# pelinski/TransformerGrooveInfilling

Hardware: AMD Instinct MI355X
Metric: HVO sequences/sec (32-step, d_model=128) per train step (higher is better)
Workload: dtype f32; 1 GPU; BASELINE configs[1]: InfillingClosedHH_training.yaml + overrides d_model=128/4 heads/3 layers, dim_feedforward=512, bs=64 per GPU, dropout=0.24, SGD lr=0.07, hit_loss_penalty=0.38, S=16, encoder-only; global_batch=64, parallelism=dp1, hipgraph=False

## Files before the change

### transformergrooveinfilling_amd/csrc/gt_seq.h

```cpp
#pragma once
#include "gt_seq_api.h"
#include <type_traits>

#ifdef GT_SEQ_STAMPS
#define GT_STAMP(i) do { if (blockIdx.x == 0 && threadIdx.x == 0) reinterpret_cast<long long*>(a.ws + a.stamps)[(i)] = (long long)__builtin_amdgcn_s_memtime(); } while (0)
__shared__ long long* gt_sub_ptr;
#define GT_SUBSTAMP(i) do { if (threadIdx.x == 0 && gt_sub_ptr) gt_sub_ptr[(i)] = (long long)__builtin_amdgcn_s_memtime(); } while (0)
#define GT_SUBWAIT() asm volatile("s_waitcnt vmcnt(0) lgkmcnt(0)" ::: "memory")
#define GT_SUBSET(on) do { if (threadIdx.x == 0) gt_sub_ptr = ((on) && blockIdx.x == 0) ? reinterpret_cast<long long*>(a.ws + a.stamps) + 200 : nullptr; } while (0)
#define GT_WGSTAMP(k) do { if (threadIdx.x == 0 && a.phase == 1 && blockIdx.x < 512) { long long* q_ = reinterpret_cast<long long*>(a.ws + a.stamps) + 1024 + 4 * blockIdx.x + 2 * (k); \
    q_[0] = (long long)__builtin_amdgcn_s_memtime(); q_[1] = (long long)__builtin_amdgcn_s_memrealtime(); } } while (0)
#else
#define GT_WGSTAMP(k) do { } while (0)
#define GT_STAMP(i) do { } while (0)
#define GT_SUBSTAMP(i) do { } while (0)
#define GT_SUBWAIT() do { } while (0)
#define GT_SUBSET(on) do { } while (0)
#endif

#define GT_SEQ_WAVES 8
#define GT_SEQ_NT (GT_SEQ_WAVES * 64)
#define GT_SEQ_NT_WG GT_SEQ_NT
#include "gt_seq_wg.h"

// ... 478 lines not shown
  const int q4 = ncol >> 2;
  for (int e = tid; e < nrows * q4; e += GT_SEQ_NT) {
    const int r = rb + e / q4, c = (e % q4) * 4;
    *reinterpret_cast<float4*>(dst + (unsigned)(r * ncol + c)) = *reinterpret_cast<const float4*>(sT + r * str + c);
  }
}

__device__ __forceinline__ void seq_tile_out_cols(float* __restrict__ dst, const int ldd, const float* sT, const int str, const int c0, const int ncol,
                                                  const int tid, const int rb, const int nrows) {
  const int q4 = ncol >> 2;
  for (int e = tid; e < nrows * q4; e += GT_SEQ_NT) {
    const int r = rb + e / q4, c = c0 + (e % q4) * 4;
    *reinterpret_cast<float4*>(dst + (unsigned)(r * ldd + c)) = *reinterpret_cast<const float4*>(sT + r * str + c);
  }
}

template <int CW> struct SeqLnPre { float ga[CW], be[CW], bi[CW]; };
template <int CW>
__device__ __forceinline__ void seq_ln_pre(SeqLnPre<CW>& p, const float* __restrict__ bias, const float* __restrict__ gamma, const float* __restrict__ beta,
                                           const int tid) {
  const int c0 = (tid & 15) * CW;
  SeqVec<CW>::ld(p.ga, gamma + c0); SeqVec<CW>::ld(p.be, beta + c0); SeqVec<CW>::ld(p.bi, bias + c0);
}
template <int DP, bool HALF, typename ZFun>
__device__ __forceinline__ void seq_ln_fwd(ZFun zfun, float* sY, const int str, const int d, const float* __restrict__ gamma,
                                           const float* __restrict__ beta, float* gy, float* gxhat, float* grstd, const int tid, const int rb,
                                           const SeqLnPre<DP / 16>* pre = nullptr) {
  constexpr int CW = DP / 16;
  if (HALF && tid >= 256) return;
  const int row = rb + (tid >> 4), seg = tid & 15, c0 = seg * CW;
  const bool ok = c0 < d;
  float z[CW], ga[CW], be[CW];
#pragma unroll
  for (int e = 0; e < CW; ++e) { z[e] = 0.f; ga[e] = 0.f; be[e] = 0.f; }
  if (ok) {
    if (pre != nullptr) {
#pragma unroll
      for (int e = 0; e < CW; ++e) { ga[e] = pre->ga[e]; be[e] = pre->be[e]; }
    } else { SeqVec<CW>::ld(ga, gamma + c0); SeqVec<CW>::ld(be, beta + c0); }
    zfun(row, c0, z);
  }
  float s = 0.f;
#pragma unroll
  for (int e = 0; e < CW; ++e) s += z[e];
  const float invd = 1.0f / (float)d, mean = seq_row16_sum(s) * invd;
  float q = 0.f;
  if (ok) {
#pragma unroll
    for (int e = 0; e < CW; ++e) { const float t = z[e] - mean; q += t * t; }
  }
  const float rs = 1.0f / sqrtf(seq_row16_sum(q) * invd + GT_LN_EPS);
  if (ok) {
    float xh[CW], y[CW];
#pragma unroll
    for (int e = 0; e < CW; ++e) { xh[e] = (z[e] - mean) * rs; y[e] = xh[e] * ga[e] + be[e]; }
    const unsigned o = (unsigned)(row * d + c0);
    SeqVec<CW>::st(sY + row * str + c0, y);
    if (gy != nullptr) {
      SeqVec<CW>::st(gy + o, y);
      SeqVec<CW>::st(gxhat + o, xh);
    }
  }
  if (seg == 0 && gy != nullptr) grstd[row] = rs;
}

template <int CW> struct SeqLnBwdPre { float xh[CW], ga[CW], rs; };
template <int CW>
__device__ __forceinline__ void seq_ln_bwd_pre(SeqLnBwdPre<CW>& p, const int d, const float* __restrict__ gxhat, const float* __restrict__ grstd,
                                               const float* __restrict__ gamma, const int tid, const int rb) {
  const int row = rb + ((tid >> 4) & 15), c0 = (tid & 15) * CW;
  SeqVec<CW>::ld(p.xh, gxhat + (unsigned)(row * d + c0)); SeqVec<CW>::ld(p.ga, gamma + c0);
  p.rs = grstd[row];
}
template <int DP, bool HALF, typename GFun>
__device__ __forceinline__ void seq_ln_bwd(GFun gfun, float* sDz, float* sDzm, const int str, const int d, const float* __restrict__ gxhat,
                                           const float* __restrict__ grstd, const float* __restrict__ gamma, const SeqDropK& dk, const uint32_t key,
                                           const uint32_t idx0, float* gdz, float* gdzm, float* sP, const int tid, const int rb,
                                           const SeqLnBwdPre<DP / 16>* pre = nullptr) {
  constexpr int CW = DP / 16;
  if (HALF && tid >= 256) return;
  const int row = rb + (tid >> 4), seg = tid & 15, c0 = seg * CW, lane = tid & 63, wave = tid >> 6;
  const bool ok = c0 < d;
  const unsigned o = (unsigned)(row * d + c0);
  float g[CW], xh[CW], ga[CW];
#pragma unroll
  for (int e = 0; e < CW; ++e) { g[e] = 0.f; xh[e] = 0.f; ga[e] = 0.f; }
  float rs;
  if (pre != nullptr) {
    rs = pre->rs;
#pragma unroll
    for (int e = 0; e < CW; ++e) { xh[e] = pre->xh[e]; ga[e] = pre->ga[e]; }
    if (ok) gfun(row, c0, g);
  } else {
    rs = grstd[row];
    if (ok) { SeqVec<CW>::ld(xh, gxhat + o); SeqVec<CW>::ld(ga, gamma + c0); gfun(row, c0, g); }
  }
  float s1 = 0.f, s2 = 0.f;
#pragma unroll
  for (int e = 0; e < CW; ++e) { const float gd = g[e] * ga[e]; s1 += gd; s2 += gd * xh[e]; }
  const float invd = 1.0f / (float)d, m1 = seq_row16_sum(s1) * invd, m2 = seq_row16_sum(s2) * invd;
  float cg[CW], cb[CW];
#pragma unroll
  for (int e = 0; e < CW; ++e) { cg[e] = g[e] * xh[e]; cb[e] = g[e]; }
#pragma unroll
  for (int e = 0; e < CW; ++e) { cg[e] += __shfl_xor(cg[e], 16); cb[e] += __shfl_xor(cb[e], 16); }
#pragma unroll
  for (int e = 0; e < CW; ++e) { cg[e] += __shfl_xor(cg[e], 32); cb[e] += __shfl_xor(cb[e], 32); }
  if (lane < 16 && ok) { SeqVec<CW>::st(sP + (wave * 2) * DP + c0, cg); SeqVec<CW>::st(sP + (wave * 2 + 1) * DP + c0, cb); }
  if (ok) {
    float v[CW], vm[CW];
// ... 461 lines not shown
#pragma unroll
    for (int c = 0; c < HD; ++c) sQ[ia * ldq + ha * HD + c] = G.dq.v[c];
  }
  if (tid < 2 * nkrow * H) {
    const int pb = tid & 1, jb = krow0 + (tid >> 1) % nkrow, hb = (tid >> 1) / nkrow;
    float* dst = sQ + jb * ldq + (pb ? 2 * d : d) + hb * HD;
#pragma unroll
    for (int c = 0; c < HD; ++c) dst[c] = pb ? G.dvv.v[c] : G.dkk.v[c];
  }
}

__device__ __forceinline__ int seq_vblock(const int bid, const int nper, const int B) {
  if ((B & 7) != 0 || bid >= nper * B) return bid;
  const int xcd = bid & 7, slot = bid >> 3;
  return ((slot / nper) * 8 + xcd) * nper + slot % nper;
}

template <int DP> struct SeqGeo {
  static constexpr int SX = DP + 8, SH = GT_SEQ_FMAX + 8, SQ = 3 * DP + 8, SRS = DP + 8, RP = DP == 32 ? 8 : DP == 64 ? 2 : 1, CW = DP / 16;
  static constexpr int TILE = 32 * SX, QKV = 32 * SQ, FFN = 32 * SH, RES = RP * 32 * SRS, NK = DP / 16;
  static constexpr int UNI = QKV > FFN ? QKV : FFN;
};
template <int DP> struct SeqFwdLds { static constexpr int N = 3 * SeqGeo<DP>::TILE + SeqGeo<DP>::RES + SeqGeo<DP>::UNI; };
template <int DP, int HDC, bool EXACT, bool SPLIT, bool QUAD = false>
__device__ __forceinline__ bool seq_fwd_body(const SeqArgs& a, float* const lds) {
  static_assert(!QUAD || (SPLIT && EXACT && DP == 128), "QUAD: the SPLIT kernels of d_model 128");
  using G = SeqGeo<DP>;
  constexpr int SX = G::SX, SH = G::SH, SQ = G::SQ, SRS = G::SRS, CW = G::CW, NK = G::NK;
  constexpr int HD = SeqHd<HDC>::HD;
  constexpr bool PAD = SeqHd<HDC>::PAD;
  constexpr bool HALF = SPLIT;
  constexpr int NH = HALF ? 1 : 2, NROW = HALF ? 16 : 32;
  float* const sX = lds; float* const sX1 = sX + G::TILE; float* const sC = sX1 + G::TILE; float* const sR = sC + G::TILE; float* const sU = sR + G::RES;
  float* const sQ = sU;
  float* const sH = sU;
  const int tid = threadIdx.x, lane = tid & 63, wave = tid >> 6, l16 = lane & 15, lg = lane >> 4;
  const int vb = (SPLIT && !QUAD) ? seq_vblock((int)blockIdx.x, 2, a.B) : (int)blockIdx.x;
  const int cpart = QUAD ? (vb & 1) : 0;
  const int half_id = QUAD ? (vb >> 1) : vb;
  const int b = SPLIT ? half_id >> 1 : (int)blockIdx.x, rb = SPLIT ? 16 * (half_id & 1) : 0;
  const bool sv0 = !QUAD || cpart == 0, sv1 = !QUAD || cpart == 1;
  const int d = EXACT ? DP : a.d, F = a.F;
  const size_t r0 = (size_t)b * 32;
  const float* const zp = gt_zero_ptr();
  const float* prm = a.prm;
  float* ws = a.ws;
  const SeqDropK dk = seq_dropk(a);
  const uint32_t idxd = (uint32_t)(r0 * d), idxf = (uint32_t)(r0 * F);
  const float ascale = 1.0f / sqrtf((float)a.hd);
// ... 68 lines not shown
        const int col = d + n0 + 4 * lg;
        *reinterpret_cast<float4*>(&sQ[l16 * SQ + col]) = make_float4(c0[0] + bi.x, c0[1] + bi.y, c0[2] + bi.z, c0[3] + bi.w);
        *reinterpret_cast<float4*>(&sQ[(16 + l16) * SQ + col]) = make_float4(c1[0] + bi.x, c1[1] + bi.y, c1[2] + bi.z, c1[3] + bi.w);
      });
    } else {
      seq_mm_tiles<NK, (3 * DP / 16 + 7) / 8, EXACT, HF>(sX + rbx * SX, SX, d, kf, 3 * d, pl + a.p0.in_b, wave, lane,
                                                          [&](int n0, const f32x4& c0, const f32x4& c1, const float4& bi) {
        const int col = n0 + 4 * lg;
        *reinterpret_cast<float4*>(&sQ[(rbx + l16) * SQ + col]) = make_float4(c0[0] + bi.x, c0[1] + bi.y, c0[2] + bi.z, c0[3] + bi.w);
        if (!HF) *reinterpret_cast<float4*>(&sQ[(16 + l16) * SQ + col]) = make_float4(c1[0] + bi.x, c1[1] + bi.y, c1[2] + bi.z, c1[3] + bi.w);
      }, PF32 && HF && have_ipre, ipre, &ipre_b);
      have_ipre = false;
    }
    GT_BARRIER();
    GT_STAMP(2 + 10 * l + 1);
  };
  auto layer_rest = [&](const int l, const bool save_qkv) -> bool {
    const float* pl = prm + (int64_t)l * a.pstride;
    const float* kf = ws + a.pack_f + (int64_t)l * a.kstride;
    const float* kf_out = kf + 3 * d * d, *kf_w1 = kf + 4 * d * d, *kf_w2 = kf_w1 + d * F;
    float* wl = ws + (int64_t)l * a.wstride;
    const int site0 = GT_SITE_LAYER0 + 8 * l;
    const int sb = 2 + 10 * l;
    const bool fzl = QUAD && a.fuse_b0 != 0 && l + 1 == a.L;
    if (save_qkv && sv0) seq_tile_out(wl + a.w0.qkv + r0 * 3 * d, sQ, SQ, 3 * d, tid, rb, NROW);
    SeqLnPre<CW> ln1p, ln2p;
    if constexpr (PFLN) seq_ln_pre<CW>(ln1p, pl + a.p0.out_b, pl + a.p0.n1w, pl + a.p0.n1b, tid);
    const bool preo = SPLIT && EXACT && (DP > 64 || PF32);
    SeqB<NK> bopre = SeqB<NK>();
    if (preo) bopre = seq_tiles_first<NK>(kf_out, d, d, wave, lane);
    bool vattn = false;
    if constexpr (PAD && SPLIT && (DP == 32 || DP == 64)) {
      vattn = a.hd == DP / 16 && a.H == 16;
      if (vattn) {
        const uint32_t key = seq_key(dk, site0 + GT_SITE_ATTN);
        float* Pseq = wl + a.w0.P + (size_t)(b * a.H) * 1024;
        const uint32_t pseq = (uint32_t)(b * a.H * 1024);
        seq_attn_fwd_small<DP / 16>(sQ, SQ, d, a.H, ascale, Pseq, pseq, sC, SX, dk, key, reinterpret_cast<uint32_t*>(ws + a.amask + (int64_t)l * a.amask_stride) + b * a.H * 32, rb, NROW, tid);
      }
    }
    if (!vattn) {
      const uint32_t key = seq_key(dk, site0 + GT_SITE_ATTN);
      constexpr int HPR = HALF ? GT_SEQ_WAVES : GT_SEQ_WAVES / 2;
      for (int h4 = 0; h4 < a.H; h4 += HPR) {
        const int h = h4 + (HALF ? wave : wave >> 1);
        if (h < a.H) {
          SeqAttn at;
// ... 2 lines not shown
          seq_attn_fwd<HD, PAD>(at, sC + h * a.hd, SX, dk, key, HALF ? (rb >> 4) : (wave & 1), lane);
        }
      }
    }
    GT_BARRIER();
    GT_STAMP(sb + 2);
    constexpr int F1T = GT_SEQ_FMAX / (QUAD ? 256 : 128);
    SeqTilesAll<NK, F1T> f1p;
    if constexpr (PF32) seq_tiles_all_load<NK, F1T>(f1p, kf_w1, d, F, pl + a.p0.b1, wave, lane);
    {
      if (sv1) seq_tile_out(wl + a.w0.ctx + r0 * d, sC, SX, d, tid, rb, NROW);
      if (DP <= 64 && !SPLIT) seq_mm_square(sC, SX, d, kf_out, sR, SRS, wave, lane);
      else
        seq_mm_tiles<NK, 1, EXACT, HALF>(sC + rb * SX, SX, d, kf_out, d, nullptr, wave, lane, [&](int n0, const f32x4& c0, const f32x4& c1, const float4&) {
          *reinterpret_cast<float4*>(&sR[(rb + l16) * SRS + n0 + 4 * lg]) = make_float4(c0[0], c0[1], c0[2], c0[3]);
          if (!HALF) *reinterpret_cast<float4*>(&sR[(16 + l16) * SRS + n0 + 4 * lg]) = make_float4(c1[0], c1[1], c1[2], c1[3]);
        }, preo, bopre);
    }
    GT_BARRIER();
    GT_STAMP(sb + 3);
    {
      const uint32_t key = seq_key(dk, site0 + GT_SITE_DROP1);
      const float* bo = pl + a.p0.out_b;
      seq_ln_fwd<DP, HALF>([&](int row, int c0, float (&z)[CW]) {
        float bi[CW], xr[CW];
        SeqVec<CW>::ld(z, &sR[row * SRS + c0]); SeqVec<CW>::ld(xr, &sX[row * SX + c0]);
        if constexpr (PFLN) {
#pragma unroll
          for (int e = 0; e < CW; ++e) bi[e] = ln1p.bi[e];
        } else SeqVec<CW>::ld(bi, bo + c0);
#pragma unroll
        for (int e = 0; e < CW; ++e) z[e] = (z[e] + bi[e]) * seq_dmul(dk, key, idxd + (uint32_t)(row * d + c0 + e)) + xr[e];
      }, sX1, SX, d, pl + a.p0.n1w, pl + a.p0.n1b, (sv1 || fzl) ? wl + a.w0.x1 + r0 * d : nullptr, wl + a.w0.xhat1 + r0 * d, wl + a.w0.rstd1 + r0, tid, rb,
         PFLN ? &ln1p : nullptr);
    }
    GT_BARRIER();
    GT_STAMP(sb + 4);
    const int fc0 = QUAD ? cpart * (F >> 1) : 0, fcn = QUAD ? F >> 1 : F;
    if constexpr (PFLN) seq_ln_pre<CW>(ln2p, pl + a.p0.b2, pl + a.p0.n2w, pl + a.p0.n2b, tid);
    if constexpr (PF32) {
      if (l + 1 < a.L) {
        const float* kfn = ws + a.pack_f + (int64_t)(l + 1) * a.kstride;
        const int tcl = wave < (3 * d >> 4) ? wave : 0;
        seq_b_load<NK, true>(ipre, kfn, d >> 4, tcl, 0, d >> 4, lane);
        ipre_b = *reinterpret_cast<const float4*>(prm + (int64_t)(l + 1) * a.pstride + a.p0.in_b + 16 * tcl + 4 * lg);
        have_ipre = true;
      }
    }
    {
      const uint32_t key = seq_key(dk, site0 + GT_SITE_FFN);
      GT_SUBSET(l == 1);
      auto ffn1_epi = [&](int n0, const f32x4& c0, const f32x4& c1, const float4& bi) {
        const int col = fc0 + n0 + 4 * lg;
#pragma unroll
        for (int h2 = 0; h2 < NH; ++h2) {
          const int row = rb + 16 * h2 + l16;
          const f32x4& c = h2 ? c1 : c0;
// ... 6 lines not shown
          *reinterpret_cast<float4*>(&sH[row * SH + col]) = v;
        }
      };
      if constexpr (PF32) seq_mm_tiles_all<NK, F1T, HALF>(sX1 + rb * SX, SX, d, fcn, wave, lane, f1p, ffn1_epi);
      else seq_mm_tiles<NK, F1T, EXACT, HALF>(sX1 + rb * SX, SX, d, kf_w1 + (size_t)(fc0 >> 4) * (d >> 4) * 256, fcn, pl + a.p0.b1 + fc0, wave, lane, ffn1_epi);
    }
    const int nkf = F >> 4, kq0 = QUAD ? cpart * (nkf >> 1) : 0;
    const bool pre2 = QUAD ? ((nkf >> 1) & 7) == 0 : (SPLIT && seq_splitk_pre_ok(F, d));
    SeqB<8> b2pre = SeqB<8>();
    if (pre2) {
      if (QUAD) seq_b_load<8, true>(b2pre, kf_w2, nkf, wave, kq0, 8, lane);
      else b2pre = seq_splitk_first(kf_w2, F, d, wave, lane);
    }
    GT_BARRIER();
    GT_SUBSET(false);
    GT_STAMP(sb + 5);
    if constexpr (QUAD) {
      seq_tile_out_cols(wl + a.w0.hact + r0 * F, F, sH, SH, fc0, fcn, tid, rb, NROW);
      f32x4 acc0 = f32x4{0.f, 0.f, 0.f, 0.f}, acc1 = acc0;
      seq_mm_krange<true>(acc0, acc1, sH + rb * SH + l16 * SH + 4 * lg, SH, kf_w2, nkf, wave, kq0, kq0 + (nkf >> 1), lane, pre2, b2pre);
      GT_STAMP(300 + 4 * l);
      unsigned long long* const xq = reinterpret_cast<unsigned long long*>(ws + a.xchg) + 8;
      const bool last = l + 1 == a.L;
      const bool fz = a.fuse_b0 != 0;
      if (!last || cpart == 1 || fz) seq_xchg_put(xq + (size_t)vb * GT_XCHG_WG_GRANULES, acc0, tid);
      if (last && cpart == 1 && !fz) return true;
      *reinterpret_cast<float4*>(&sR[(16 * cpart + l16) * SRS + 16 * wave + 4 * lg]) = make_float4(acc0[0], acc0[1], acc0[2], acc0[3]);
      GT_STAMP(301 + 4 * l);
      const f32x4 oth = seq_xchg_get(xq + (size_t)(vb ^ 1) * GT_XCHG_WG_GRANULES, tid, reinterpret_cast<unsigned*>(ws + a.xchg), a.spin_max);
      GT_STAMP(302 + 4 * l);
      *reinterpret_cast<float4*>(&sR[(16 * (1 - cpart) + l16) * SRS + 16 * wave + 4 * lg]) = make_float4(oth[0], oth[1], oth[2], oth[3]);
    } else {
      seq_tile_out(wl + a.w0.hact + r0 * F, sH, SH, F, tid, rb, NROW);
      seq_mm_splitk<HALF>(sH + rb * SH, SH, F, kf_w2, d, sR + rb * SRS, SRS, wave, lane, pre2, b2pre);
    }
    GT_BARRIER();
    GT_STAMP(sb + 6);
    {
      const uint32_t key = seq_key(dk, site0 + GT_SITE_DROPF);
      const float* b2 = pl + a.p0.b2;
      const int parts = seq_splitk_parts(d);
      seq_ln_fwd<DP, HALF>([&](int row, int c0, float (&z)[CW]) {
        float bi[CW], xr[CW];
        if constexpr (QUAD) {
          float u[CW];
          SeqVec<CW>::ld(z, &sR[(row - rb) * SRS + c0]); SeqVec<CW>::ld(u, &sR[(16 + row - rb) * SRS + c0]);
#pragma unroll
          for (int e = 0; e < CW; ++e) z[e] += u[e];
        } else {
          seq_parts_sum<CW>(z, sR, SRS, parts, row, c0);
        }
        SeqVec<CW>::ld(xr, &sX1[row * SX + c0]);
        if constexpr (PFLN) {
#pragma unroll
          for (int e = 0; e < CW; ++e) bi[e] = ln2p.bi[e];
        } else SeqVec<CW>::ld(bi, b2 + c0);
#pragma unroll
        for (int e = 0; e < CW; ++e) z[e] = (z[e] + bi[e]) * seq_dmul(dk, key, idxd + (uint32_t)(row * d + c0 + e)) + xr[e];
      }, sX, SX, d, pl + a.p0.n2w, pl + a.p0.n2b, (sv0 || fzl) ? wl + a.w0.xout + r0 * d : nullptr, wl + a.w0.xhat2 + r0 * d, wl + a.w0.rstd2 + r0, tid, rb,
         PFLN ? &ln2p : nullptr);
    }
    GT_BARRIER();
    GT_STAMP(sb + 7);
    return false;
  };
  auto output_layer = [&]() {
    seq_ln_fwd<DP, HALF>([&](int row, int c0, float (&z)[CW]) { SeqVec<CW>::ld(z, &sX[row * SX + c0]); }, sC, SX, d, prm + a.encn_w, prm + a.encn_b,
                         ws + a.memory + r0 * d, ws + a.enc_xhat + r0 * d, ws + a.enc_rstd + r0, tid, rb);
    GT_BARRIER();
    seq_mm_edge<false, true, NK, HALF>(sC + rb * SX, SX, d, prm + a.out_w, d, GT_TGT, prm + a.out_b, wave, lane, zp,
                                       [&](int n0, const f32x4& c0, const f32x4& c1, const float (&bi)[4]) {
#pragma unroll
      for (int h2 = 0; h2 < NH; ++h2) {
        const f32x4& c = h2 ? c1 : c0;
#pragma unroll
        for (int r = 0; r < 4; ++r) {
          const int col = n0 + 4 * lg + r;
          if (col < GT_TGT) {
            float v = c[r] + bi[r];
            if (col >= 2 * GT_VOICES) v = 0.5f * tanhf(v);
            else if (col >= GT_VOICES) v = gt_sigmoid(v);
            a.hvo[(r0 + rb + 16 * h2 + l16) * GT_TGT + col] = v;
            sR[(rb + 16 * h2 + l16) * 28 + col] = v;
          }
        }
      }
    });
    if (a.loss_y == nullptr) return;
    const unsigned lwg_n = QUAD ? gridDim.x >> 1 : gridDim.x, lwg_id = QUAD ? (unsigned)half_id : blockIdx.x;
    GT_BARRIER();
    float* red = sX1;
    const float invM = 1.0f / (float)(a.B * 32);
    float bce = 0.f, mv = 0.f, mo = 0.f, ok = 0.f;
    if (tid < NROW * GT_VOICES) {
      const int row = rb + tid / GT_VOICES, j = tid % GT_VOICES;
      const size_t base = (r0 + row) * GT_TGT + j;
      float gh, gv, go;
      gt_loss_elem<true>(sR[row * 28 + j], sR[row * 28 + j + GT_VOICES], sR[row * 28 + j + 2 * GT_VOICES], a.loss_y[base],
                         a.loss_y[base + GT_VOICES], a.loss_y[base + 2 * GT_VOICES], a.loss_penalty, invM, bce, mv, mo, ok, gh, gv, go);
      ws[a.dlogits + base] = gh; ws[a.dlogits + base + GT_VOICES] = gv; ws[a.dlogits + base + 2 * GT_VOICES] = go;
    }
    bce = gt_wave_sum(bce); mv = gt_wave_sum(mv); mo = gt_wave_sum(mo); ok = gt_wave_sum(ok);
    if (lane == 0) { red[wave * 4 + 0] = bce; red[wave * 4 + 1] = mv; red[wave * 4 + 2] = mo; red[wave * 4 + 3] = ok; }
    GT_BARRIER();
    if (tid == 0 && cpart != 0) red[32] = 0.0f;
    if (tid == 0 && cpart == 0) {
#pragma unroll
      for (int q = 0; q < 4; ++q) {
        float t = red[q];
        for (int w = 1; w < GT_SEQ_WAVES; ++w) t += red[w * 4 + q];
        gt_pub_store(a.loss_part + lwg_id * 4 + q, t);
      }
      const unsigned t = gt_pub_ticket(a.loss_ticket);
      red[32] = (t == lwg_n - 1) ? 1.0f : 0.0f;
    }
    GT_BARRIER();
    if (red[32] == 0.0f) return;
    if (wave < 4) {
      float acc = 0.f;
      for (unsigned bk = lane; bk < lwg_n; bk += 64) acc += gt_pub_load(a.loss_part + bk * 4 + wave);
      acc = gt_wave_sum(acc);
      if (lane == 0) red[40 + wave] = acc * invM;
    }
    GT_BARRIER();
    if (tid == 0) {
      const float b_ = red[40], v_ = red[41], o_ = red[42];
      a.loss_stats[0] = b_ + v_ + o_;
// ... 49 lines not shown
      GT_BARRIER();
    }
    GT_STAMP(2 + 10 * l + 1);
    if (layer_rest(l, l == 0 && !pro)) return false;
    if (l + 1 < a.L) {
      in_proj(l + 1, OwnRows{});
      float* const gq = ws + (int64_t)(l + 1) * a.wstride + a.w0.qkv + r0 * 3 * d;
      if (QUAD) seq_tile_out_cols(gq, 3 * d, sQ, SQ, cpart * (3 * d / 2), 3 * d / 2, tid, rb, NROW);
      else seq_tile_out(gq, sQ, SQ, 3 * d, tid, rb, NROW);
    } else {
      output_layer();
    }
    GT_WGSTAMP(1);
    GT_STAMP(61 + 2 * (l + 1));
  }
  return true;
}
template <int DP, int HDC, bool EXACT, bool SPLIT, bool QUAD = false>
__global__ __launch_bounds__(GT_SEQ_NT) void seq_fwd_kernel(SeqArgs a) {
  __shared__ __attribute__((aligned(16))) float lds[SeqFwdLds<DP>::N];
  (void)seq_fwd_body<DP, HDC, EXACT, SPLIT, QUAD>(a, lds);
}

template <int DP> struct SeqBwdLds {
  using G = SeqGeo<DP>;
  static constexpr int U = DP > 64 ? G::UNI : G::QKV + G::FFN, P = 2 * GT_SEQ_WAVES * DP;
  static constexpr int N = 3 * G::TILE + G::RES + U + P + 32 * GT_SEQ_WAVES / 2;
};
template <int DP, int HDC, bool EXACT, bool SPLIT, bool QUAD = false>
__device__ __forceinline__ void seq_bwd_body(const SeqArgs& a, float* const lds) {
  static_assert(!QUAD || (SPLIT && EXACT && DP == 128), "QUAD: the SPLIT kernels of d_model 128");
  using G = SeqGeo<DP>;
  constexpr int SX = G::SX, SH = G::SH, SQ = G::SQ, SRS = G::SRS, CW = G::CW, NK = G::NK;
  constexpr int HD = SeqHd<HDC>::HD;
  constexpr bool PAD = SeqHd<HDC>::PAD;
  constexpr bool HALF = SPLIT;
  constexpr int NROW = HALF ? 16 : 32;
  constexpr bool ALIAS = DP > 64;
  float* const sZ = lds; float* const sDZ = sZ + G::TILE; float* const sC = sDZ + G::TILE; float* const sR = sC + G::TILE;
  float* const sU = sR + G::RES; float* const sP = sU + SeqBwdLds<DP>::U; float* const srd = sP + SeqBwdLds<DP>::P;
  float* const sQ = sU;
  float* const sH = ALIAS ? sU : sU + G::QKV;
  const int tid = threadIdx.x, lane = tid & 63, wave = tid >> 6, l16 = lane & 15, lg = lane >> 4;
  const int vb = (SPLIT && !QUAD) ? seq_vblock((int)blockIdx.x, 2, a.B) : (int)blockIdx.x;
  const int cpart = QUAD ? (vb & 1) : 0, half_id = QUAD ? (vb >> 1) : vb;
  const int b = SPLIT ? half_id >> 1 : (int)blockIdx.x, rb = SPLIT ? 16 * (half_id & 1) : 0;
  const bool sv0 = !QUAD || cpart == 0;
  const int d = EXACT ? DP : a.d, F = a.F;
  const size_t r0 = (size_t)b * 32;
  if constexpr (SPLIT && DP == 128 && !QUAD) {
    if (a.grd != nullptr && (int)blockIdx.x >= a.nseq) {
      static_assert(SeqBwdLds<DP>::U >= GT_WG_LDS && SeqBwdLds<DP>::P >= 8 * 64, "rider LDS");
      seq_wg_riders(a, a.phase, (int)blockIdx.x - a.nseq, (int)gridDim.x - a.nseq, sU, sP, tid);
      return;
    }
  }
  const float* const zp = gt_zero_ptr();
  const float* prm = a.prm;
  float* ws = a.ws;
  const SeqDropK dk = seq_dropk(a);
  const uint32_t idxd = (uint32_t)(r0 * d);
  const float mscale = dk.thr ? dk.scale : 1.0f;
  const float ascale = 1.0f / sqrtf((float)a.hd);
  auto part_at = [&](int job) { return ws + a.ln_part + (int64_t)job * a.ln_part_stride + (size_t)(QUAD ? half_id : (int)blockIdx.x) * 2 * d; };
  auto load_rows = [&](float* dst, const int str, const float* src, const int ncol, const int rb_, const int nrows) {
    const int q4 = ncol >> 2;
    for (int e = tid; e < nrows * q4; e += GT_SEQ_NT) {
      const int r = rb_ + e / q4, c = (e % q4) * 4;
      *reinterpret_cast<float4*>(dst + r * str + c) = *reinterpret_cast<const float4*>(src + (unsigned)(r * ncol + c));
    }
  };

  auto prologue = [&]() {
    for (int e = tid; e < NROW * 32; e += GT_SEQ_NT) {
      const int r = rb + (e >> 5), c = e & 31;
      sC[r * SX + c] = *(c < GT_TGT ? ws + a.dlogits + (r0 + r) * GT_TGT + c : zp);
    }
    if (!SPLIT) load_rows(sH, SH, ws + a.w0.hact + (int64_t)(a.L - 1) * a.wstride + r0 * F, F, 0, 32);
    GT_BARRIER();
    seq_mm_edge<true, true, 2, HALF>(sC + rb * SX, SX, GT_TGT, prm + a.out_w, d, d, nullptr, wave, lane, zp,
                                     [&](int n0, const f32x4& c0, const f32x4& c1, const float (&)[4]) {
      const int col = n0 + 4 * lg;
      *reinterpret_cast<float4*>(&sZ[(rb + l16) * SX + col]) = make_float4(c0[0], c0[1], c0[2], c0[3]);
      if (!HALF) *reinterpret_cast<float4*>(&sZ[(16 + l16) * SX + col]) = make_float4(c1[0], c1[1], c1[2], c1[3]);
    });
    GT_BARRIER();
    {
      SeqDropK nd = dk; nd.thr = 0u;
      seq_ln_bwd<DP, HALF>([&](int row, int c0, float (&g)[CW]) { SeqVec<CW>::ld(g, &sZ[row * SX + c0]); }, sZ, sC, SX, d, ws + a.enc_xhat + r0 * d,
                           ws + a.enc_rstd + r0, prm + a.encn_w, nd, 0u, 0u, nullptr, nullptr, sP, tid, rb);
    }
    GT_BARRIER();
    if (sv0) seq_ln_part<DP, HALF>(sP, part_at(0), d, tid);
    GT_BARRIER();
    GT_STAMP(101);
  };
  constexpr bool PFB = SPLIT && !QUAD && EXACT && (DP == 32 || DP == 64);
  constexpr bool PFBLN = PFB;
  SeqLnBwdPre<CW> lb2p, lb1p;
  bool have_lbp = false;
  constexpr int F2T = GT_SEQ_FMAX / (QUAD ? 256 : 128);
  SeqTilesAll<NK, F2T> f2p;
  auto chain = [&](const int l, const bool fromg) {
    const float* pl = prm + (int64_t)l * a.pstride;
    const float* kb = ws + a.pack_b + (int64_t)l * a.kstride;
    const float* kb_out = kb + 3 * d * d, *kb_w1 = kb + 4 * d * d, *kb_w2 = kb_w1 + d * F;
    float* wl = ws + (int64_t)l * a.wstride;
    float* tl = ws + (int64_t)l * a.tstride;
    const int site0 = GT_SITE_LAYER0 + 8 * l, jb = 1 + 2 * (a.L - 1 - l);
    const int sb = 102 + 10 * (a.L - 1 - l);
    static_assert(16 * GT_SEQ_FMAX / 4 <= 4 * GT_SEQ_NT, "four 16-byte loads per thread cover the 16 x F tile");
    if constexpr (PFB) seq_tiles_all_load<NK, F2T, false>(f2p, kb_w2, d, F, nullptr, wave, lane);
    float4 hp0 = make_float4(0.f, 0.f, 0.f, 0.f), hp1 = hp0, hp2 = hp0, hp3 = hp0;
    const int fc0 = QUAD ? cpart * (F >> 1) : 0, fcn = QUAD ? F >> 1 : F;
    const int hq4 = fcn >> 2, hn = 16 * hq4;
    auto hoff = [&](const int u) { const int e = tid + u * GT_SEQ_NT, ec = e < hn ? e : hn - 1; return (unsigned)((rb + ec / hq4) * F + fc0 + (ec % hq4) * 4); };
    if (SPLIT) {
      const float* src = wl + a.w0.hact + r0 * F;
      hp0 = *reinterpret_cast<const float4*>(src + hoff(0)); hp1 = *reinterpret_cast<const float4*>(src + hoff(1));
      hp2 = *reinterpret_cast<const float4*>(src + hoff(2)); hp3 = *reinterpret_cast<const float4*>(src + hoff(3));
    } else if (ALIAS && !fromg) {
      load_rows(sH, SH, wl + a.w0.hact + r0 * F, F, rb, NROW);
    }
    {
      const uint32_t key = seq_key(dk, site0 + GT_SITE_DROPF);
      const int parts = seq_splitk_parts(d);
      seq_ln_bwd<DP, HALF>([&](int row, int c0, float (&g)[CW]) {
        if (fromg) SeqVec<CW>::ld(g, &sZ[row * SX + c0]);
        else {
          float r[CW];
          seq_parts_sum<CW>(g, sR, SRS, parts, row, c0); SeqVec<CW>::ld(r, &sDZ[row * SX + c0]);
#pragma unroll
          for (int e = 0; e < CW; ++e) g[e] += r[e];
        }
      }, sDZ, sC, SX, d, wl + a.w0.xhat2 + r0 * d, wl + a.w0.rstd2 + r0, pl + a.p0.n2w, dk, key, idxd, sv0 ? tl + a.t0.dzA + r0 * d : nullptr,
                           (dk.thr && sv0) ? tl + a.t0.dzAm + r0 * d : nullptr, sP, tid, rb, (PFBLN && have_lbp) ? &lb2p : nullptr);
    }
    if (SPLIT) {
      auto hst = [&](const int u, const float4& v) { const int e = tid + u * GT_SEQ_NT; if (e < hn) *reinterpret_cast<float4*>(sH + (rb + e / hq4) * SH + fc0 + (e % hq4) * 4) = v; };
      hst(0, hp0); hst(1, hp1); hst(2, hp2); hst(3, hp3);
    }
    GT_BARRIER();
    GT_STAMP(sb);
    if (sv0) seq_ln_part<DP, HALF>(sP, part_at(jb), d, tid);
    auto ffn2d_epi = [&](int n0, const f32x4& c0, const f32x4& c1, const float4&) {
      const int col = fc0 + n0 + 4 * lg;
#pragma unroll
      for (int h2 = 0; h2 < (HALF ? 1 : 2); ++h2) {
        float* hp = &sH[(rb + 16 * h2 + l16) * SH + col];
        const f32x4& c = h2 ? c1 : c0;
        const float4 ha = *reinterpret_cast<const float4*>(hp);
        *reinterpret_cast<float4*>(hp) = make_float4(ha.x != 0.f ? c[0] * mscale : 0.f, ha.y != 0.f ? c[1] * mscale : 0.f,
                                                     ha.z != 0.f ? c[2] * mscale : 0.f, ha.w != 0.f ? c[3] * mscale : 0.f);
      }
    };
    if constexpr (PFB) seq_mm_tiles_all<NK, F2T, HALF>(sC + rb * SX, SX, d, fcn, wave, lane, f2p, ffn2d_epi);
    else seq_mm_tiles<NK, F2T, EXACT, HALF>(sC + rb * SX, SX, d, kb_w2 + (size_t)(fc0 >> 4) * (d >> 4) * 256, fcn, nullptr, wave, lane, ffn2d_epi);
    const int nkf = F >> 4, kq0 = QUAD ? cpart * (nkf >> 1) : 0;
    const bool pre1 = QUAD ? ((nkf >> 1) & 7) == 0 : (SPLIT && seq_splitk_pre_ok(F, d));
    SeqB<8> b1pre = SeqB<8>();
    if (pre1) {
      if (QUAD) seq_b_load<8, true>(b1pre, kb_w1, nkf, wave, kq0, 8, lane);
      else b1pre = seq_splitk_first(kb_w1, F, d, wave, lane);
    }
    GT_BARRIER();
    GT_STAMP(sb + 1);
    SeqB<NK> bodpre = SeqB<NK>();
    if constexpr (PFB) bodpre = seq_tiles_first<NK>(kb_out, d, d, wave, lane);
    if constexpr (QUAD) {
      seq_tile_out_cols(tl + a.t0.dhid + r0 * F, F, sH, SH, fc0, fcn, tid, rb, NROW);
      f32x4 acc0 = f32x4{0.f, 0.f, 0.f, 0.f}, acc1 = acc0;
      seq_mm_krange<true>(acc0, acc1, sH + rb * SH + l16 * SH + 4 * lg, SH, kb_w1, nkf, wave, kq0, kq0 + (nkf >> 1), lane, pre1, b1pre);
      const int64_t xoff = a.fuse_b0 ? a.xchg_b : a.xchg;
      unsigned long long* const xq = reinterpret_cast<unsigned long long*>(ws + xoff) + 8;
      seq_xchg_put(xq + (size_t)vb * GT_XCHG_WG_GRANULES, acc0, tid);
      *reinterpret_cast<float4*>(&sR[(16 * cpart + l16) * SRS + 16 * wave + 4 * lg]) = make_float4(acc0[0], acc0[1], acc0[2], acc0[3]);
      const f32x4 oth = seq_xchg_get(xq + (size_t)(vb ^ 1) * GT_XCHG_WG_GRANULES, tid, reinterpret_cast<unsigned*>(ws + a.xchg), a.spin_max);
      *reinterpret_cast<float4*>(&sR[(16 * (1 - cpart) + l16) * SRS + 16 * wave + 4 * lg]) = make_float4(oth[0], oth[1], oth[2], oth[3]);
    } else {
      seq_tile_out(tl + a.t0.dhid + r0 * F, sH, SH, F, tid, rb, NROW);
      seq_mm_splitk<HALF>(sH + rb * SH, SH, F, kb_w1, d, sR + rb * SRS, SRS, wave, lane, pre1, b1pre);
    }
    GT_BARRIER();
    GT_STAMP(sb + 2);
    if (!SPLIT) load_rows(sQ, SQ, wl + a.w0.qkv + r0 * 3 * d, 3 * d, 0, 32);
    {
      const uint32_t key = seq_key(dk, site0 + GT_SITE_DROP1);
      const int parts = seq_splitk_parts(d);
      seq_ln_bwd<DP, HALF>([&](int row, int c0, float (&g)[CW]) {
        float r[CW];
        if constexpr (QUAD) {
          float u[CW];
          SeqVec<CW>::ld(g, &sR[(row - rb) * SRS + c0]); SeqVec<CW>::ld(u, &sR[(16 + row - rb) * SRS + c0]);
#pragma unroll
          for (int e = 0; e < CW; ++e) g[e] += u[e];
        } else {
          seq_parts_sum<CW>(g, sR, SRS, parts, row, c0);
        }
        SeqVec<CW>::ld(r, &sDZ[row * SX + c0]);
#pragma unroll
        for (int e = 0; e < CW; ++e) g[e] += r[e];
      }, sDZ, sC, SX, d, wl + a.w0.xhat1 + r0 * d, wl + a.w0.rstd1 + r0, pl + a.p0.n1w, dk, key, idxd, sv0 ? tl + a.t0.dzB + r0 * d : nullptr,
                           (dk.thr && sv0) ? tl + a.t0.dzBm + r0 * d : nullptr, sP, tid, rb, (PFBLN && have_lbp) ? &lb1p : nullptr);
    }
    GT_BARRIER();
    GT_STAMP(sb + 3);
    if (sv0) seq_ln_part<DP, HALF>(sP, part_at(jb + 1), d, tid);
    if (DP <= 64 && !SPLIT) seq_mm_square(sC, SX, d, kb_out, sZ, SX, wave, lane);
    else if constexpr (QUAD)
      seq_mm_tiles<NK, 1, EXACT, true>(sC + rb * SX, SX, d, kb_out + (size_t)cpart * (d >> 5) * NK * 256, d >> 1, nullptr, wave, lane,
                                       [&](int n0, const f32x4& c0, const f32x4&, const float4&) {
        *reinterpret_cast<float4*>(&sZ[(rb + l16) * SX + cpart * (d >> 1) + n0 + 4 * lg]) = make_float4(c0[0], c0[1], c0[2], c0[3]);
      });
    else
      seq_mm_tiles<NK, 1, EXACT, HALF>(sC + rb * SX, SX, d, kb_out, d, nullptr, wave, lane, [&](int n0, const f32x4& c0, const f32x4& c1, const float4&) {
        *reinterpret_cast<float4*>(&sZ[(rb + l16) * SX + n0 + 4 * lg]) = make_float4(c0[0], c0[1], c0[2], c0[3]);
        if (!HALF) *reinterpret_cast<float4*>(&sZ[(16 + l16) * SX + n0 + 4 * lg]) = make_float4(c1[0], c1[1], c1[2], c1[3]);
      }, PFB, bodpre);
    GT_BARRIER();
    GT_STAMP(sb + 4);
  };
  auto chain_prefetch = [&](const int l) {
    if constexpr (PFBLN) {
      if (l > 0) {
        const float* wp = ws + (int64_t)(l - 1) * a.wstride;
        const float* pp = prm + (int64_t)(l - 1) * a.pstride;
// ... 98 lines not shown
                                       reinterpret_cast<const uint32_t*>(ws + a.amask + (int64_t)l * a.amask_stride) + b * a.H * 32, tid);
    }
    load_rows(sZ, SX, ws + a.dctx + ((a.phase - 1) & 1) * hand + r0 * d, d, 0, 32);
    load_rows(sQ, SQ, ws + (int64_t)l * a.wstride + a.w0.qkv + r0 * 3 * d, 3 * d, 0, 32);
    load_rows(sDZ, SX, ws + (int64_t)l * a.tstride + a.t0.dzB + r0 * d, d, rb, NROW);
    chain_prefetch(l);
    GT_BARRIER();
    GT_STAMP(400 + 4 * a.phase);
    attn_inproj(l);
    if (l > 0) {
      chain(l - 1, false);
      seq_tile_out(ws + a.dctx + (a.phase & 1) * hand + r0 * d, sZ, SX, d, tid, rb, NROW);
    } else {
      input_bwd();
    }
    GT_STAMP(161 + 2 * a.phase);
  }
}
template <int DP, int HDC, bool EXACT, bool SPLIT, bool QUAD = false>
__global__ __launch_bounds__(GT_SEQ_NT) void seq_bwd_kernel(SeqArgs a) {
  __shared__ __attribute__((aligned(16))) float lds[SeqBwdLds<DP>::N];
  seq_bwd_body<DP, HDC, EXACT, SPLIT, QUAD>(a, lds);
}
template <int HDC>
__global__ __launch_bounds__(GT_SEQ_NT) void seq_fb_kernel(SeqArgs a) {
  constexpr int N = SeqBwdLds<128>::N > SeqFwdLds<128>::N ? SeqBwdLds<128>::N : SeqFwdLds<128>::N;
  __shared__ __attribute__((aligned(16))) float lds[N];
  if (!seq_fwd_body<128, HDC, true, true, true>(a, lds)) return;
  __syncthreads();
  SeqArgs b = a;
  b.phase = 0;
  seq_bwd_body<128, 32, true, true, true>(b, lds);
}
```

Measured before the change: 323,200 sequences/s.

## Keep forward LN stats and logit grads in LDS across fused fwd-bwd kernel

In the fused forward+backward kernel, the forward LayerNorms now stash xhat and rstd into LDS rows that the backward reads directly instead of reloading from global memory. Output logit gradients are written straight into the backward's A tile, and the FFN hidden activations are left in place in shared memory rather than reloaded. The loss reduction ticket is moved after the backward so it no longer blocks the phase change. Together these aim to cut global round-trips and one barrier per step, but they depend on careful LDS aliasing (row^16 halves, shared offsets) and add some complexity.

```diff
diff --git a/transformergrooveinfilling_amd/csrc/gt_seq.h b/transformergrooveinfilling_amd/csrc/gt_seq.h
--- a/transformergrooveinfilling_amd/csrc/gt_seq.h
+++ b/transformergrooveinfilling_amd/csrc/gt_seq.h
@@ -524,10 +524,10 @@
   const int c0 = (tid & 15) * CW;
   SeqVec<CW>::ld(p.ga, gamma + c0); SeqVec<CW>::ld(p.be, beta + c0); SeqVec<CW>::ld(p.bi, bias + c0);
 }
-template <int DP, bool HALF, typename ZFun>
+template <int DP, bool HALF, bool STASH = false, typename ZFun>
 __device__ __forceinline__ void seq_ln_fwd(ZFun zfun, float* sY, const int str, const int d, const float* __restrict__ gamma,
                                            const float* __restrict__ beta, float* gy, float* gxhat, float* grstd, const int tid, const int rb,
-                                           const SeqLnPre<DP / 16>* pre = nullptr) {
+                                           const SeqLnPre<DP / 16>* pre = nullptr, float* sS = nullptr) {
   constexpr int CW = DP / 16;
   if (HALF && tid >= 256) return;
   const int row = rb + (tid >> 4), seg = tid & 15, c0 = seg * CW;
@@ -562,8 +562,15 @@
       SeqVec<CW>::st(gy + o, y);
       SeqVec<CW>::st(gxhat + o, xh);
     }
+    if constexpr (STASH) SeqVec<CW>::st(sS + (row ^ 16) * str + c0, xh);
   }
   if (seg == 0 && gy != nullptr) grstd[row] = rs;
+  if constexpr (STASH) { if (seg == 0) sS[(row ^ 16) * str + DP] = rs; }
+}
+template <int DP>
+__device__ __forceinline__ void seq_ln_stash_ld(const float* sS, const int str, const int row, const int c0, float (&xh)[DP / 16], float& rs) {
+  SeqVec<DP / 16>::ld(xh, sS + (row ^ 16) * str + c0);
+  rs = sS[(row ^ 16) * str + DP];
 }
 
 template <int CW> struct SeqLnBwdPre { float xh[CW], ga[CW], rs; };
@@ -574,11 +581,11 @@
   SeqVec<CW>::ld(p.xh, gxhat + (unsigned)(row * d + c0)); SeqVec<CW>::ld(p.ga, gamma + c0);
   p.rs = grstd[row];
 }
-template <int DP, bool HALF, typename GFun>
+template <int DP, bool HALF, typename GFun, typename XFun = std::nullptr_t>
 __device__ __forceinline__ void seq_ln_bwd(GFun gfun, float* sDz, float* sDzm, const int str, const int d, const float* __restrict__ gxhat,
                                            const float* __restrict__ grstd, const float* __restrict__ gamma, const SeqDropK& dk, const uint32_t key,
                                            const uint32_t idx0, float* gdz, float* gdzm, float* sP, const int tid, const int rb,
-                                           const SeqLnBwdPre<DP / 16>* pre = nullptr) {
+                                           const SeqLnBwdPre<DP / 16>* pre = nullptr, XFun xfun = XFun()) {
   constexpr int CW = DP / 16;
   if (HALF && tid >= 256) return;
   const int row = rb + (tid >> 4), seg = tid & 15, c0 = seg * CW, lane = tid & 63, wave = tid >> 6;
@@ -588,6 +595,10 @@
 #pragma unroll
   for (int e = 0; e < CW; ++e) { g[e] = 0.f; xh[e] = 0.f; ga[e] = 0.f; }
   float rs;
+  if constexpr (!std::is_same<XFun, std::nullptr_t>::value) {
+    rs = 0.f;
+    if (ok) { SeqVec<CW>::ld(ga, gamma + c0); xfun(row, c0, xh, rs); gfun(row, c0, g); }
+  } else
   if (pre != nullptr) {
     rs = pre->rs;
 #pragma unroll
@@ -1095,9 +1106,15 @@
   static constexpr int UNI = QKV > FFN ? QKV : FFN;
 };
 template <int DP> struct SeqFwdLds { static constexpr int N = 3 * SeqGeo<DP>::TILE + SeqGeo<DP>::RES + SeqGeo<DP>::UNI; };
-template <int DP, int HDC, bool EXACT, bool SPLIT, bool QUAD = false>
+template <int DP> struct SeqBwdLds {
+  using G = SeqGeo<DP>;
+  static constexpr int U = DP > 64 ? G::UNI : G::QKV + G::FFN, P = 2 * GT_SEQ_WAVES * DP;
+  static constexpr int N = 3 * G::TILE + G::RES + U + P + 32 * GT_SEQ_WAVES / 2;
+};
+template <int DP, int HDC, bool EXACT, bool SPLIT, bool QUAD = false, bool FUSED = false>
 __device__ __forceinline__ bool seq_fwd_body(const SeqArgs& a, float* const lds) {
   static_assert(!QUAD || (SPLIT && EXACT && DP == 128), "QUAD: the SPLIT kernels of d_model 128");
+  static_assert(!FUSED || QUAD, "FUSED: the QUAD schedule");
   using G = SeqGeo<DP>;
   constexpr int SX = G::SX, SH = G::SH, SQ = G::SQ, SRS = G::SRS, CW = G::CW, NK = G::NK;
   constexpr int HD = SeqHd<HDC>::HD;
@@ -1212,7 +1229,7 @@
     float* wl = ws + (int64_t)l * a.wstride;
     const int site0 = GT_SITE_LAYER0 + 8 * l;
     const int sb = 2 + 10 * l;
-    const bool fzl = QUAD && a.fuse_b0 != 0 && l + 1 == a.L;
+    const bool fzl = QUAD && !FUSED && a.fuse_b0 != 0 && l + 1 == a.L;
     if (save_qkv && sv0) seq_tile_out(wl + a.w0.qkv + r0 * 3 * d, sQ, SQ, 3 * d, tid, rb, NROW);
     SeqLnPre<CW> ln1p, ln2p;
     if constexpr (PFLN) seq_ln_pre<CW>(ln1p, pl + a.p0.out_b, pl + a.p0.n1w, pl + a.p0.n1b, tid);
@@ -1261,7 +1278,7 @@
     {
       const uint32_t key = seq_key(dk, site0 + GT_SITE_DROP1);
       const float* bo = pl + a.p0.out_b;
-      seq_ln_fwd<DP, HALF>([&](int row, int c0, float (&z)[CW]) {
+      seq_ln_fwd<DP, HALF, FUSED>([&](int row, int c0, float (&z)[CW]) {
         float bi[CW], xr[CW];
         SeqVec<CW>::ld(z, &sR[row * SRS + c0]); SeqVec<CW>::ld(xr, &sX[row * SX + c0]);
         if constexpr (PFLN) {
@@ -1271,7 +1288,7 @@
 #pragma unroll
         for (int e = 0; e < CW; ++e) z[e] = (z[e] + bi[e]) * seq_dmul(dk, key, idxd + (uint32_t)(row * d + c0 + e)) + xr[e];
       }, sX1, SX, d, pl + a.p0.n1w, pl + a.p0.n1b, (sv1 || fzl) ? wl + a.w0.x1 + r0 * d : nullptr, wl + a.w0.xhat1 + r0 * d, wl + a.w0.rstd1 + r0, tid, rb,
-         PFLN ? &ln1p : nullptr);
+         PFLN ? &ln1p : nullptr, sX1);
     }
     GT_BARRIER();
     GT_STAMP(sb + 4);
@@ -1324,7 +1341,7 @@
       GT_STAMP(300 + 4 * l);
       unsigned long long* const xq = reinterpret_cast<unsigned long long*>(ws + a.xchg) + 8;
       const bool last = l + 1 == a.L;
-      const bool fz = a.fuse_b0 != 0;
+      const bool fz = FUSED || a.fuse_b0 != 0;
       if (!last || cpart == 1 || fz) seq_xchg_put(xq + (size_t)vb * GT_XCHG_WG_GRANULES, acc0, tid);
       if (last && cpart == 1 && !fz) return true;
       *reinterpret_cast<float4*>(&sR[(16 * cpart + l16) * SRS + 16 * wave + 4 * lg]) = make_float4(acc0[0], acc0[1], acc0[2], acc0[3]);
@@ -1342,7 +1359,7 @@
       const uint32_t key = seq_key(dk, site0 + GT_SITE_DROPF);
       const float* b2 = pl + a.p0.b2;
       const int parts = seq_splitk_parts(d);
-      seq_ln_fwd<DP, HALF>([&](int row, int c0, float (&z)[CW]) {
+      seq_ln_fwd<DP, HALF, FUSED>([&](int row, int c0, float (&z)[CW]) {
         float bi[CW], xr[CW];
         if constexpr (QUAD) {
           float u[CW];
@@ -1360,16 +1377,17 @@
 #pragma unroll
         for (int e = 0; e < CW; ++e) z[e] = (z[e] + bi[e]) * seq_dmul(dk, key, idxd + (uint32_t)(row * d + c0 + e)) + xr[e];
       }, sX, SX, d, pl + a.p0.n2w, pl + a.p0.n2b, (sv0 || fzl) ? wl + a.w0.xout + r0 * d : nullptr, wl + a.w0.xhat2 + r0 * d, wl + a.w0.rstd2 + r0, tid, rb,
-         PFLN ? &ln2p : nullptr);
+         PFLN ? &ln2p : nullptr, sX);
     }
     GT_BARRIER();
     GT_STAMP(sb + 7);
     return false;
   };
   auto output_layer = [&]() {
-    seq_ln_fwd<DP, HALF>([&](int row, int c0, float (&z)[CW]) { SeqVec<CW>::ld(z, &sX[row * SX + c0]); }, sC, SX, d, prm + a.encn_w, prm + a.encn_b,
-                         ws + a.memory + r0 * d, ws + a.enc_xhat + r0 * d, ws + a.enc_rstd + r0, tid, rb);
-    GT_BARRIER();
+    seq_ln_fwd<DP, HALF, FUSED>([&](int row, int c0, float (&z)[CW]) { SeqVec<CW>::ld(z, &sX[row * SX + c0]); }, sC, SX, d, prm + a.encn_w, prm + a.encn_b,
+                                (!FUSED || sv0) ? ws + a.memory + r0 * d : nullptr, ws + a.enc_xhat + r0 * d, ws + a.enc_rstd + r0, tid, rb, nullptr, sC);
+    GT_BARRIER();
+    GT_STAMP(500);
     seq_mm_edge<false, true, NK, HALF>(sC + rb * SX, SX, d, prm + a.out_w, d, GT_TGT, prm + a.out_b, wave, lane, zp,
                                        [&](int n0, const f32x4& c0, const f32x4& c1, const float (&bi)[4]) {
 #pragma unroll
@@ -1382,7 +1400,7 @@
             float v = c[r] + bi[r];
             if (col >= 2 * GT_VOICES) v = 0.5f * tanhf(v);
             else if (col >= GT_VOICES) v = gt_sigmoid(v);
-            a.hvo[(r0 + rb + 16 * h2 + l16) * GT_TGT + col] = v;
+            if (!FUSED || sv0) a.hvo[(r0 + rb + 16 * h2 + l16) * GT_TGT + col] = v;
             sR[(rb + 16 * h2 + l16) * 28 + col] = v;
           }
         }
@@ -1391,7 +1409,8 @@
     if (a.loss_y == nullptr) return;
     const unsigned lwg_n = QUAD ? gridDim.x >> 1 : gridDim.x, lwg_id = QUAD ? (unsigned)half_id : blockIdx.x;
     GT_BARRIER();
-    float* red = sX1;
+    GT_STAMP(501);
+    float* red = FUSED ? lds + SeqFwdLds<DP>::N + SeqBwdLds<DP>::P : sX1;
     const float invM = 1.0f / (float)(a.B * 32);
     float bce = 0.f, mv = 0.f, mo = 0.f, ok = 0.f;
     if (tid < NROW * GT_VOICES) {
@@ -1400,11 +1419,19 @@
       float gh, gv, go;
       gt_loss_elem<true>(sR[row * 28 + j], sR[row * 28 + j + GT_VOICES], sR[row * 28 + j + 2 * GT_VOICES], a.loss_y[base],
                          a.loss_y[base + GT_VOICES], a.loss_y[base + 2 * GT_VOICES], a.loss_penalty, invM, bce, mv, mo, ok, gh, gv, go);
-      ws[a.dlogits + base] = gh; ws[a.dlogits + base + GT_VOICES] = gv; ws[a.dlogits + base + 2 * GT_VOICES] = go;
+      if constexpr (FUSED) {
+        static_assert(32 - GT_TGT <= GT_VOICES, "the row's voice threads zero the A tile's padding columns");
+        float* sd = sC + row * SX + j;
+        sd[0] = gh; sd[GT_VOICES] = gv; sd[2 * GT_VOICES] = go;
+        if (j < 32 - GT_TGT) sd[GT_TGT] = 0.f;
+      }
+      if (!FUSED || sv0) { ws[a.dlogits + base] = gh; ws[a.dlogits + base + GT_VOICES] = gv; ws[a.dlogits + base + 2 * GT_VOICES] = go; }
     }
     bce = gt_wave_sum(bce); mv = gt_wave_sum(mv); mo = gt_wave_sum(mo); ok = gt_wave_sum(ok);
     if (lane == 0) { red[wave * 4 + 0] = bce; red[wave * 4 + 1] = mv; red[wave * 4 + 2] = mo; red[wave * 4 + 3] = ok; }
     GT_BARRIER();
+    GT_STAMP(502);
+    if constexpr (FUSED) return;
     if (tid == 0 && cpart != 0) red[32] = 0.0f;
     if (tid == 0 && cpart == 0) {
 #pragma unroll
@@ -1500,14 +1527,10 @@
   (void)seq_fwd_body<DP, HDC, EXACT, SPLIT, QUAD>(a, lds);
 }
 
-template <int DP> struct SeqBwdLds {
-  using G = SeqGeo<DP>;
-  static constexpr int U = DP > 64 ? G::UNI : G::QKV + G::FFN, P = 2 * GT_SEQ_WAVES * DP;
-  static constexpr int N = 3 * G::TILE + G::RES + U + P + 32 * GT_SEQ_WAVES / 2;
-};
-template <int DP, int HDC, bool EXACT, bool SPLIT, bool QUAD = false>
+template <int DP, int HDC, bool EXACT, bool SPLIT, bool QUAD = false, bool FUSED = false>
 __device__ __forceinline__ void seq_bwd_body(const SeqArgs& a, float* const lds) {
   static_assert(!QUAD || (SPLIT && EXACT && DP == 128), "QUAD: the SPLIT kernels of d_model 128");
+  static_assert(!FUSED || QUAD, "FUSED: phase 0 of the QUAD schedule");
   using G = SeqGeo<DP>;
   constexpr int SX = G::SX, SH = G::SH, SQ = G::SQ, SRS = G::SRS, CW = G::CW, NK = G::NK;
   constexpr int HD = SeqHd<HDC>::HD;
@@ -1515,6 +1538,8 @@
   constexpr bool HALF = SPLIT;
   constexpr int NROW = HALF ? 16 : 32;
   constexpr bool ALIAS = DP > 64;
+  static_assert(!FUSED || (ALIAS && SeqFwdLds<DP>::N - G::UNI == 3 * G::TILE + G::RES),
+                "FUSED: the forward's FFN tile and this body's sH are one place (same offset, same stride SH)");
   float* const sZ = lds; float* const sDZ = sZ + G::TILE; float* const sC = sDZ + G::TILE; float* const sR = sC + G::TILE;
   float* const sU = sR + G::RES; float* const sP = sU + SeqBwdLds<DP>::U; float* const srd = sP + SeqBwdLds<DP>::P;
   float* const sQ = sU;
@@ -1549,13 +1574,19 @@
     }
   };
 
+  auto stash_of = [&](const float* sS) {
+    if constexpr (FUSED) return [sS](int row, int c0, float (&xh)[CW], float& rs) { seq_ln_stash_ld<DP>(sS, SX, row, c0, xh, rs); };
+    else return nullptr;
+  };
   auto prologue = [&]() {
-    for (int e = tid; e < NROW * 32; e += GT_SEQ_NT) {
-      const int r = rb + (e >> 5), c = e & 31;
-      sC[r * SX + c] = *(c < GT_TGT ? ws + a.dlogits + (r0 + r) * GT_TGT + c : zp);
-    }
-    if (!SPLIT) load_rows(sH, SH, ws + a.w0.hact + (int64_t)(a.L - 1) * a.wstride + r0 * F, F, 0, 32);
-    GT_BARRIER();
+    if constexpr (!FUSED) {
+      for (int e = tid; e < NROW * 32; e += GT_SEQ_NT) {
+        const int r = rb + (e >> 5), c = e & 31;
+        sC[r * SX + c] = *(c < GT_TGT ? ws + a.dlogits + (r0 + r) * GT_TGT + c : zp);
+      }
+      if (!SPLIT) load_rows(sH, SH, ws + a.w0.hact + (int64_t)(a.L - 1) * a.wstride + r0 * F, F, 0, 32);
+      GT_BARRIER();
+    }
     seq_mm_edge<true, true, 2, HALF>(sC + rb * SX, SX, GT_TGT, prm + a.out_w, d, d, nullptr, wave, lane, zp,
                                      [&](int n0, const f32x4& c0, const f32x4& c1, const float (&)[4]) {
       const int col = n0 + 4 * lg;
@@ -1563,12 +1594,14 @@
       if (!HALF) *reinterpret_cast<float4*>(&sZ[(16 + l16) * SX + col]) = make_float4(c1[0], c1[1], c1[2], c1[3]);
     });
     GT_BARRIER();
+    GT_STAMP(503);
     {
       SeqDropK nd = dk; nd.thr = 0u;
       seq_ln_bwd<DP, HALF>([&](int row, int c0, float (&g)[CW]) { SeqVec<CW>::ld(g, &sZ[row * SX + c0]); }, sZ, sC, SX, d, ws + a.enc_xhat + r0 * d,
-                           ws + a.enc_rstd + r0, prm + a.encn_w, nd, 0u, 0u, nullptr, nullptr, sP, tid, rb);
-    }
-    GT_BARRIER();
+                           ws + a.enc_rstd + r0, prm + a.encn_w, nd, 0u, 0u, nullptr, nullptr, sP, tid, rb, nullptr, stash_of(sC));
+    }
+    GT_BARRIER();
+    GT_STAMP(504);
     if (sv0) seq_ln_part<DP, HALF>(sP, part_at(0), d, tid);
     GT_BARRIER();
     GT_STAMP(101);
@@ -1593,12 +1626,14 @@
     const int fc0 = QUAD ? cpart * (F >> 1) : 0, fcn = QUAD ? F >> 1 : F;
     const int hq4 = fcn >> 2, hn = 16 * hq4;
     auto hoff = [&](const int u) { const int e = tid + u * GT_SEQ_NT, ec = e < hn ? e : hn - 1; return (unsigned)((rb + ec / hq4) * F + fc0 + (ec % hq4) * 4); };
+    if constexpr (!FUSED) {
     if (SPLIT) {
       const float* src = wl + a.w0.hact + r0 * F;
       hp0 = *reinterpret_cast<const float4*>(src + hoff(0)); hp1 = *reinterpret_cast<const float4*>(src + hoff(1));
       hp2 = *reinterpret_cast<const float4*>(src + hoff(2)); hp3 = *reinterpret_cast<const float4*>(src + hoff(3));
     } else if (ALIAS && !fromg) {
       load_rows(sH, SH, wl + a.w0.hact + r0 * F, F, rb, NROW);
+    }
     }
     {
       const uint32_t key = seq_key(dk, site0 + GT_SITE_DROPF);
@@ -1612,11 +1647,13 @@
           for (int e = 0; e < CW; ++e) g[e] += r[e];
         }
       }, sDZ, sC, SX, d, wl + a.w0.xhat2 + r0 * d, wl + a.w0.rstd2 + r0, pl + a.p0.n2w, dk, key, idxd, sv0 ? tl + a.t0.dzA + r0 * d : nullptr,
-                           (dk.thr && sv0) ? tl + a.t0.dzAm + r0 * d : nullptr, sP, tid, rb, (PFBLN && have_lbp) ? &lb2p : nullptr);
-    }
+                           (dk.thr && sv0) ? tl + a.t0.dzAm + r0 * d : nullptr, sP, tid, rb, (PFBLN && have_lbp) ? &lb2p : nullptr, stash_of(sZ));
+    }
+    if constexpr (!FUSED) {
     if (SPLIT) {
       auto hst = [&](const int u, const float4& v) { const int e = tid + u * GT_SEQ_NT; if (e < hn) *reinterpret_cast<float4*>(sH + (rb + e / hq4) * SH + fc0 + (e % hq4) * 4) = v; };
       hst(0, hp0); hst(1, hp1); hst(2, hp2); hst(3, hp3);
+    }
     }
     GT_BARRIER();
     GT_STAMP(sb);
@@ -1649,7 +1686,8 @@
       seq_tile_out_cols(tl + a.t0.dhid + r0 * F, F, sH, SH, fc0, fcn, tid, rb, NROW);
       f32x4 acc0 = f32x4{0.f, 0.f, 0.f, 0.f}, acc1 = acc0;
       seq_mm_krange<true>(acc0, acc1, sH + rb * SH + l16 * SH + 4 * lg, SH, kb_w1, nkf, wave, kq0, kq0 + (nkf >> 1), lane, pre1, b1pre);
-      const int64_t xoff = a.fuse_b0 ? a.xchg_b : a.xchg;
+      int64_t xoff = a.fuse_b0 ? a.xchg_b : a.xchg;
+      if constexpr (FUSED) xoff = a.xchg_b;
       unsigned long long* const xq = reinterpret_cast<unsigned long long*>(ws + xoff) + 8;
       seq_xchg_put(xq + (size_t)vb * GT_XCHG_WG_GRANULES, acc0, tid);
       *reinterpret_cast<float4*>(&sR[(16 * cpart + l16) * SRS + 16 * wave + 4 * lg]) = make_float4(acc0[0], acc0[1], acc0[2], acc0[3]);
@@ -1679,7 +1717,7 @@
 #pragma unroll
         for (int e = 0; e < CW; ++e) g[e] += r[e];
       }, sDZ, sC, SX, d, wl + a.w0.xhat1 + r0 * d, wl + a.w0.rstd1 + r0, pl + a.p0.n1w, dk, key, idxd, sv0 ? tl + a.t0.dzB + r0 * d : nullptr,
-                           (dk.thr && sv0) ? tl + a.t0.dzBm + r0 * d : nullptr, sP, tid, rb, (PFBLN && have_lbp) ? &lb1p : nullptr);
+                           (dk.thr && sv0) ? tl + a.t0.dzBm + r0 * d : nullptr, sP, tid, rb, (PFBLN && have_lbp) ? &lb1p : nullptr, stash_of(sDZ));
     }
     GT_BARRIER();
     GT_STAMP(sb + 3);
@@ -1824,13 +1862,46 @@
   __shared__ __attribute__((aligned(16))) float lds[SeqBwdLds<DP>::N];
   seq_bwd_body<DP, HDC, EXACT, SPLIT, QUAD>(a, lds);
 }
+__device__ __forceinline__ void seq_fb_ticket(const SeqArgs& a, float* red, const unsigned lwg_n, const unsigned lwg_id, const float invM, const int tid) {
+  const int lane = tid & 63, wave = tid >> 6;
+  if (tid == 0) {
+#pragma unroll
+    for (int q = 0; q < 4; ++q) {
+      float t = red[q];
+      for (int w = 1; w < GT_SEQ_WAVES; ++w) t += red[w * 4 + q];
+      gt_pub_store(a.loss_part + lwg_id * 4 + q, t);
+    }
+    const unsigned t = gt_pub_ticket(a.loss_ticket);
+    red[32] = (t == lwg_n - 1) ? 1.0f : 0.0f;
+  }
+  GT_BARRIER();
+  if (red[32] == 0.0f) return;
+  if (wave < 4) {
+    float acc = 0.f;
+    for (unsigned bk = lane; bk < lwg_n; bk += 64) acc += gt_pub_load(a.loss_part + bk * 4 + wave);
+    acc = gt_wave_sum(acc);
+    if (lane == 0) red[40 + wave] = acc * invM;
+  }
+  GT_BARRIER();
+  if (tid == 0) {
+    const float b_ = red[40], v_ = red[41], o_ = red[42];
+    a.loss_stats[0] = b_ + v_ + o_;
+    a.loss_stats[1] = red[43] * (1.0f / GT_VOICES);
+    a.loss_stats[2] = 0.f;
+    a.loss_stats[3] = b_; a.loss_stats[4] = v_; a.loss_stats[5] = o_; a.loss_stats[6] = 0.f; a.loss_stats[7] = 0.f;
+    *a.loss_ticket = 0u;
+  }
+}
 template <int HDC>
 __global__ __launch_bounds__(GT_SEQ_NT) void seq_fb_kernel(SeqArgs a) {
   constexpr int N = SeqBwdLds<128>::N > SeqFwdLds<128>::N ? SeqBwdLds<128>::N : SeqFwdLds<128>::N;
   __shared__ __attribute__((aligned(16))) float lds[N];
-  if (!seq_fwd_body<128, HDC, true, true, true>(a, lds)) return;
-  __syncthreads();
+  if (!seq_fwd_body<128, HDC, true, true, true, true>(a, lds)) return;
   SeqArgs b = a;
   b.phase = 0;
-  seq_bwd_body<128, 32, true, true, true>(b, lds);
-}
+  seq_bwd_body<128, 32, true, true, true, true>(b, lds);
+  GT_STAMP(505);
+  if ((blockIdx.x & 1) == 0)
+    seq_fb_ticket(a, lds + SeqFwdLds<128>::N + SeqBwdLds<128>::P, gridDim.x >> 1, blockIdx.x >> 1, 1.0f / (float)(a.B * 32), (int)threadIdx.x);
+  GT_STAMP(506);
+}
```

Measured after the change: 323,000 sequences/s, median of 3. Within noise of the previous version (-0.0%).
